# arneschneuing/DiffSBDD

Hardware: AMD Instinct MI355X
Metric: sampled ligands/sec (500-step DDPM, fullatom_cond) at 1/2/4/8 MI355X (higher is better)
Workload: dtype f32

## Files before the change

### diffsbdd_amd/_lib.py

```python
from __future__ import annotations

import ctypes as C
import os

_HERE = os.path.dirname(os.path.abspath(__file__))
LIB_PATH = os.environ.get("DSBDD_LIB") or os.path.join(_HERE, "libdiffsbdd_hip.so")
ABI_VERSION = 6

OK, ERR_ARG, ERR_STATE, ERR_CAPACITY, ERR_LAUNCH = 0, -1, -2, -3, -4
STATUS_NAN, STATUS_EDGE_OVERFLOW = 1, 2

G_NAMES = ["ATOM_ENC_W0T", "ATOM_ENC_B0", "ATOM_ENC_W1T", "ATOM_ENC_B1",
           "RES_ENC_W0T", "RES_ENC_B0", "RES_ENC_W1T", "RES_ENC_B1",
           "ATOM_DEC_W0T", "ATOM_DEC_B0", "ATOM_DEC_W1T", "ATOM_DEC_B1",
           "RES_DEC_W0T", "RES_DEC_B0", "RES_DEC_W1T", "RES_DEC_B1",
           "EMB_WT", "EMB_B", "EMBOUT_WT", "EMBOUT_B"]
GCL_NAMES = ["E1_WT", "E1_WD", "E1_WD0", "E1_TAB", "E2_WT", "E2_B", "ATT_W", "ATT_B",
             "N1_WT", "N1_B", "N2_WT", "N2_B"]
EQ_NAMES = ["C1_WT", "C_WD", "C_WD0", "C_TAB", "C_W2T", "C_B2",
            "X_WD", "X_WD0", "X_TAB", "X_W2T", "X_B2", "W3"]
OPT_PRUNE, OPT_CONE, OPT_GRANULE16, OPT_EMU, OPT_SPLITK, OPT_SHELL, OPT_TAIL = 0, 1, 2, 3, 4, 5, 6
(BUF_EDGE_ROW, BUF_EDGE_COL, BUF_EDGE_D0, BUF_ROW_PTR, BUF_H, BUF_X, BUF_NODE_BATCH, BUF_DEG,
 BUF_LEVEL, BUF_LEVEL_LIST, BUF_LEVEL_COUNT, BUF_LEVEL_END, BUF_LROW_PTR, BUF_LEDGE_ROW, BUF_LEDGE_COL,
 BUF_LEDGE_D0, BUF_LEVEL_STATS) = range(17)


class Config(C.Structure):
    _fields_ = [(n, C.c_int32) for n in (
        "atom_nf", "residue_nf", "joint_nf", "hidden_nf", "n_layers", "inv_sublayers",
        "attention", "use_tanh", "update_pocket_coords", "reflection_equivariant",
        "edge_embedding_dim", "has_cutoff_ligand", "has_cutoff_pocket",
        "has_cutoff_interaction")] + [(n, C.c_float) for n in (
            "cutoff_ligand", "cutoff_pocket", "cutoff_interaction",
            "norm_constant", "normalization_factor", "coords_range")]


# ... 33 lines not shown
    "dsbdd_last_error": (C.c_char_p, []),
    "dsbdd_engine_create": (C.c_int, [C.POINTER(Config), C.POINTER(_P)]),
    "dsbdd_engine_destroy": (None, [_P]),
    "dsbdd_engine_weight_slots": (C.c_int, [_P]),
    "dsbdd_engine_set_weights": (C.c_int, [_P, C.POINTER(_P), C.c_int]),
    "dsbdd_engine_workspace_bytes": (C.c_size_t, [_P, _I64, _I64, _I64, _I64]),
    "dsbdd_engine_bind_workspace": (C.c_int, [_P, _P, C.c_size_t, _I64, _I64, _I64, _I64]),
    "dsbdd_engine_set_trace": (C.c_int, [_P, _P, _P]),
    "dsbdd_engine_set_pocket_frame": (C.c_int, [_P, _P, _P, _P, _P, _P, _I64, _I64, _I64, _I64, _I64, _I64]),
    "dsbdd_engine_clear_pocket_frame": (C.c_int, [_P]),
    "dsbdd_dynamics_forward": (C.c_int, [_P, _P, _P, _P, _P, _I64, _P, _P, _I64, _I64, _I64,
                                         _P, _P, _I64, _P, _P, _P]),
    "dsbdd_engine_buffer": (C.c_int, [_P, C.c_int, C.POINTER(_P)]),
    "dsbdd_engine_shell_read": (C.c_int, [_P, C.c_int, C.c_int, _P, C.c_int64]),
    "dsbdd_engine_graph_stats": (C.c_int, [_P, C.POINTER(_I64), C.POINTER(_I64), C.POINTER(_I64)]),
    "dsbdd_engine_last_plan": (C.c_int, [_P, C.POINTER(C.c_int32), C.POINTER(C.c_int32), C.c_int32,
                                         C.POINTER(C.c_int32), C.POINTER(C.c_int32)]),
    "dsbdd_engine_set_option": (C.c_int, [_P, C.c_int, C.c_int]),
    "dsbdd_engine_get_option": (C.c_int, [_P, C.c_int]),
    "dsbdd_engine_profile": (C.c_int, [_P, C.c_int, C.c_int]),
    "dsbdd_engine_profile_read": (C.c_int, [_P, C.POINTER(C.c_double), C.POINTER(_I64)]),
    "dsbdd_cond_reverse_update": (C.c_int, [_P, _P, _P, _P, _P, _P, _P, _I64, _I64, _I64,
                                            _I32, _I32, _F, _F, _F, _I32]),
    "dsbdd_joint_reverse_update": (C.c_int, [_P, _P, _P, _P, _P, _P, _P, _P, _P, _I64, _I64, _I64,
                                             _I32, _I32, _F, _F, _F, _I32]),
    "dsbdd_segment_mean3": (C.c_int, [_P, _P, _I32, _P, _I64, _I64, _P]),
    "dsbdd_cond_affine_noise": (C.c_int, [_P, _P, _P, _P, _P, _P, _I64, _I64, _I64, _I32, _I32, _F, _F, _I32]),
    "dsbdd_joint_affine_noise": (C.c_int, [_P, _P, _P, _P, _P, _P, _P, _I64, _I64, _I64, _I32, _I32, _F, _F,
                                           _I32, _I32]),
    "dsbdd_cond_repaint_update": (C.c_int, [_P, _P, _P, _P, _P, _P, _P, _P, _P, _P, _P, _I64, _I64, _I64,
# ... 109 lines not shown
```

### diffsbdd_amd/csrc/engine.hip

```cpp
#include "../../include/diffsbdd_hip.h"

#include <algorithm>
#include <climits>
#include <cmath>
#include <cstdio>
#include <cstdlib>
#include <cstring>
#include <string>
#include <type_traits>
#include <utility>
#include <vector>

#include "common.h"
#include "ddpm.h"
#include "edge_mlp.h"
#include "edge_wave.h"
#include "edge_wave16.h"
#include "edge_splitk.h"
#include "graph.h"
#include "lig_head.h"
#include "ligand_pack.h"
#include "molecule.h"
#include "node_chain.h"
#include "node_linear.h"
// ... 79 lines not shown
int dsbdd_engine_bind_workspace(dsbdd_engine* e, void* ws, size_t bytes, int64_t nl, int64_t np,
                                int64_t B, int64_t E) {
  if (!e || !ws) return fail(DSBDD_ERR_ARG, "null argument");
  if (reinterpret_cast<uintptr_t>(ws) & 255) return fail(DSBDD_ERR_ARG, "workspace must be 256-byte aligned");
  if ((nl + np) >= (1ll << 30) || E >= (1ll << 31) - 256) return fail(DSBDD_ERR_ARG, "problem too large for int32 indices");
  if (bytes < ws_carve(e->cfg, nl, np, B, E, nullptr).total) return fail(DSBDD_ERR_CAPACITY, "workspace too small");
  e->drop_graphs();
  static_cast<Workspace&>(*e) = ws_carve(e->cfg, nl, np, B, E, static_cast<char*>(ws));
  e->ws = static_cast<char*>(ws); e->ws_bytes = bytes;
  e->cap_lig = nl; e->cap_poc = np; e->cap_batch = B; e->cap_edges = E;
  e->cap_edgesL = 2 * E + 32 * kLevels * B;
  e->cap_tiles = e->cap_edgesL / 32 + 2;
  e->cap_shell = E + 32 * B;
  e->cap_tiles16 = e->cap_edgesL / 16 + 2;
  e->lvl_stats_zeroed = false;
  e->frame = false;
  e->ghost_dirty = true;
  e->h0_pocket_valid = false;
  e->invalidate_derived();
  return DSBDD_OK;
}

#ifdef DSBDD_TIMESTAMPS
int dsbdd_debug_set_timestamps(dsbdd_engine* e, unsigned long long* buf, int capacity) {
  if (!e) return DSBDD_ERR_ARG;
  e->ts_buf = buf; e->ts_cap = capacity; e->ts_next = 0;
  return DSBDD_OK;
}
#endif

// ... 59 lines not shown

int dsbdd_engine_set_option(dsbdd_engine* e, int which, int value) {
  if (!e) return fail(DSBDD_ERR_ARG, "null argument");
  switch (which) {
    case DSBDD_OPT_PRUNE: e->prune = value ? 1 : 0; break;
    case DSBDD_OPT_CONE: e->cone = value <= 0 ? 0 : (value >= 2 ? 2 : 1); break;
    case DSBDD_OPT_GRANULE16: e->granule16 = (unsigned)value; break;
    case DSBDD_OPT_SPLITK: e->splitk = (unsigned)value; break;
    case DSBDD_OPT_EMU:
      if (value != 0 && value != 6 && value != 9) return fail(DSBDD_ERR_ARG, "DSBDD_OPT_EMU takes 0, 6 or 9");
      e->emu = value; break;
    case DSBDD_OPT_SHELL: e->shell = value ? 1 : 0; break;
    case DSBDD_OPT_TAIL:
      if (value < 0) return fail(DSBDD_ERR_ARG, "DSBDD_OPT_TAIL takes a value >= 0");
      e->tail = value; break;
    default: return fail(DSBDD_ERR_ARG, "unknown option");
  }
  e->drop_graphs();
  return DSBDD_OK;
}

int dsbdd_engine_get_option(const dsbdd_engine* e, int which) {
  if (!e) return fail(DSBDD_ERR_ARG, "null argument");
  switch (which) {
    case DSBDD_OPT_PRUNE: return e->prune;
    case DSBDD_OPT_CONE: return e->cone;
    case DSBDD_OPT_GRANULE16: return (int)e->granule16;
    case DSBDD_OPT_SPLITK: return (int)e->splitk;
    case DSBDD_OPT_EMU: return e->emu;
    case DSBDD_OPT_SHELL: return e->shell;
    case DSBDD_OPT_TAIL: return e->tail;
  }
  return fail(DSBDD_ERR_ARG, "unknown option");
}

int dsbdd_engine_set_trace(dsbdd_engine* e, float* th, float* tx) {
  if (!e) return DSBDD_ERR_ARG;
  e->trace_h = th; e->trace_x = tx;
  return DSBDD_OK;
}

int dsbdd_engine_profile(dsbdd_engine* e, int enable, int max_launches) {
  if (!e || max_launches < 0) return fail(DSBDD_ERR_ARG, "bad argument");
  e->profile = enable < 0 ? 0 : enable;
  e->prof_call = 0;
  e->ev_used = 0;
// ... 21 lines not shown
}

int dsbdd_engine_graph_stats(const dsbdd_engine* e, int64_t* replays, int64_t* captures, int64_t* eager) {
  if (!e || !replays || !captures || !eager) return fail(DSBDD_ERR_ARG, "null argument");
  *replays = e->n_replay; *captures = e->n_capture; *eager = e->n_eager;
  return DSBDD_OK;
}

int dsbdd_engine_buffer(const dsbdd_engine* e, int which, void** out) {
  if (!e || !out || !e->ws) return fail(DSBDD_ERR_STATE, "no workspace bound");
  void* const buf[] = {e->erow, e->ecol, e->ed0, e->row_ptr, e->h, e->x, e->node_batch, e->deg, e->lvl, e->lvl_list, e->lvl_cnt,
                       e->lvl_end, e->row_ptrL, e->erowL, e->ecolL, e->ed0L, e->lvl_stats};
  static_assert(DSBDD_BUF_LEVEL_STATS + 1 == sizeof(buf) / sizeof(buf[0]), "one pointer per DSBDD_BUF_* id");
  if (which < 0 || which > DSBDD_BUF_LEVEL_STATS) return fail(DSBDD_ERR_ARG, "unknown buffer id");
  *out = buf[which];
  return DSBDD_OK;
}

int dsbdd_engine_shell_read(const dsbdd_engine* e, int which, int list, void* dst, int64_t count) {
  if (!e || !dst || count < 0) return fail(DSBDD_ERR_ARG, "bad argument");
  if (!e->shell_mem) return fail(DSBDD_ERR_STATE, "no shell stage has run on this engine");
  const int64_t N = e->shell_key[0], SL = e->shell_key[2];
  const void* src = nullptr;
  int64_t have = 0, size = 4;
  const bool lst = list >= 0 && list < kShellLists;
  switch (which) {
    case DSBDD_SHELL_STATS: src = e->sh_stats; have = 8; size = 8; break;
    case DSBDD_SHELL_COUNT: src = e->sh_cnt; have = kShellLists; break;
    case DSBDD_SHELL_ROW: if (lst) { src = e->sh_row + (size_t)list * SL; have = SL; } break;
    case DSBDD_SHELL_COL: if (lst) { src = e->sh_col + (size_t)list * SL; have = SL; } break;
// ... 41 lines not shown
```

### diffsbdd_amd/csrc/engine_state.h

```cpp
#pragma once

static thread_local std::string g_err;
static int fail(int code, const std::string& msg) { g_err = msg; return code; }

#define HIP_TRY(expr)                                                              \
  do {                                                                             \
    hipError_t _e = (expr);                                                        \
    if (_e != hipSuccess)                                                          \
      return fail(DSBDD_ERR_LAUNCH, std::string(#expr) + ": " + hipGetErrorString(_e)); \
  } while (0)
#define RC_TRY(expr)                       \
  do {                                     \
    const int _rc = (expr);                \
    if (_rc != DSBDD_OK) return _rc;       \
  } while (0)

struct StreamDevice {
  int prev = -1;
  bool switched = false;
  explicit StreamDevice(void* stream) {
    hipStream_t s = static_cast<hipStream_t>(stream);
    if (!s) return;
    hipDevice_t d = 0;
    int cur = 0;
// ... 111 lines not shown

struct dsbdd_engine : Workspace {
  dsbdd_config cfg;
  std::vector<const float*> slots;
  bool has_weights = false;
  char* ws = nullptr;
  size_t ws_bytes = 0;
  int64_t cap_lig = 0, cap_poc = 0, cap_batch = 0, cap_edges = 0;
  bool lvl_stats_zeroed = false;
  int64_t cap_edgesL = 0;
  int prune = 1;
  int cone = 1;
  int64_t ghost_slots = 0;
  int shell = 1;
  int tail = 1;
  int64_t cap_shell = 0;
  char* shell_mem = nullptr;
  int64_t shell_key[3] = {0, 0, 0};
  int *sh_seg = nullptr, *sh_deg = nullptr, *sh_ptr = nullptr, *sh_row = nullptr, *sh_col = nullptr, *sh_cnt = nullptr;
  float* sh_d0 = nullptr;
  unsigned long long* sh_stats = nullptr;
  float* msg_buf = nullptr;
  int64_t msg_cap = 0;
  std::vector<int> plan_radius, plan_ghost;
  int plan_timed_level = kLevels - 1;
  bool frame = false;
  int64_t frame_nlig = 0, frame_npoc = 0, frame_batch = 0, frame_n3 = 0, frame_cap3 = 0;
  bool ghost_dirty = true;
  bool h0_pocket_valid = false;
  int64_t cap_tiles = 0;
// ... 21 lines not shown
  struct GraphEntry {
    std::vector<uint64_t> key;
    int seen = 0;
    hipGraph_t graph = nullptr;
    hipGraphExec_t exec = nullptr;
    std::vector<int> plan_radius, plan_ghost;
    int plan_timed_level = 0;
    void destroy() { if (exec) (void)hipGraphExecDestroy(exec); if (graph) (void)hipGraphDestroy(graph); }
  };
  std::vector<GraphEntry> graphs;
  int use_graph = 1;
  int coord_split = 1;
  int node_group = 1;
  int edge_max_wg = 0;
  int64_t n_replay = 0, n_capture = 0, n_eager = 0;
  unsigned long long* ts_buf = nullptr;
  int ts_cap = 0, ts_next = 0;
  hipStream_t cap_stream = nullptr;
  dsbdd_engine() : Workspace{} {}
  void drop_graphs() {
    for (GraphEntry& g : graphs) g.destroy();
    graphs.clear();
  }
  void invalidate_derived() { derived = DerivedReady{}; }
  ~dsbdd_engine() {
    for (hipEvent_t e : ev) (void)hipEventDestroy(e);
    drop_graphs();
    if (cap_stream) (void)hipStreamDestroy(cap_stream);
    if (side_stream) (void)hipStreamDestroy(side_stream);
    if (ev_fork) (void)hipEventDestroy(ev_fork);
// ... 62 lines not shown
  const std::pair<const char*, int*> off_on_zero[] = {
      {"DSBDD_GRAPH", &e->use_graph}, {"DSBDD_EDGE_BPERM", &e->edge_bperm}, {"DSBDD_COORD_SPLIT", &e->coord_split},
      {"DSBDD_NODE_GROUP", &e->node_group}, {"DSBDD_PRUNE", &e->prune}, {"DSBDD_LIG_HEAD", &e->lig_head},
      {"DSBDD_NODE_CHAIN", &e->chain}};
  for (const auto& sw : off_on_zero) if (env_int(sw.first, &v) && v == 0) *sw.second = 0;
  const std::pair<const char*, int*> on_nonzero[] = {{"DSBDD_LEVEL_ROWS", &e->level_rows}, {"DSBDD_FORK", &e->fork_front}};
  for (const auto& sw : on_nonzero) if (env_int(sw.first, &v)) *sw.second = v != 0;
  if (env_int("DSBDD_FOLD_SCAN", &v)) e->fold_scan = v > 0 ? 1 : 0;
  if (env_int("DSBDD_GRANULE16", &v, true)) e->granule16 = (unsigned)v;
  if (env_int("DSBDD_SPLITK", &v, true)) e->splitk = (unsigned)v;
  if (env_int("DSBDD_EMU", &v)) e->emu = (v == 6 || v == 9) ? (int)v : 0;
  if (env_int("DSBDD_CONE", &v)) e->cone = v <= 0 ? 0 : (v >= 2 ? 2 : 1);
  if (env_int("DSBDD_NODE_CHAIN_MIN_ROWS", &v) && v >= 0) e->chain_min_rows = v;
  if (env_int("DSBDD_EDGE_MAX_WG", &v) && v > 0) e->edge_max_wg = (int)v;
  if (env_int("DSBDD_TAIL", &v) && v >= 0) e->tail = (int)v;
}
```

### diffsbdd_amd/csrc/forward.h

```cpp
#pragma once

struct ForwardArgs {
  const float *xh_lig, *xh_pocket, *t;
  int64_t t_count;
  const int64_t *mask_lig, *mask_pocket;
  int64_t n_lig, n_pocket, batch;
  const int32_t *ext_row, *ext_col;
  int64_t ext_n_edges;
  float *eps_lig, *eps_pocket;
  int32_t* status;
};

static bool frame_applies(const dsbdd_engine* e, const ForwardArgs& a) {
  return e->frame && !e->cfg.update_pocket_coords && !a.ext_row && a.n_lig == e->frame_nlig &&
         a.n_pocket == e->frame_npoc && a.batch == e->frame_batch;
}

static Mlp2Problem residue_encoder(const dsbdd_engine* e, const ForwardArgs& a) {
  const dsbdd_config& c = e->cfg;
  const int r = c.residue_nf, J = c.joint_nf, JP = pad4(J + 1);
  const float* const* W = e->slots.data();
  return Mlp2Problem{a.xh_pocket + 3, 3 + r, r, W[DSBDD_G_RES_ENC_W0T], pad4(2 * r), W[DSBDD_G_RES_ENC_B0], 2 * r,
                     W[DSBDD_G_RES_ENC_W1T], pad4(J), W[DSBDD_G_RES_ENC_B1], J, e->h0 + (size_t)a.n_lig * JP, JP,
                     (int)a.n_pocket};
// ... 18 lines not shown
  const int PQ = (c.reflection_equivariant ? 2 : 4) * H;
  const float* const* W = e->slots.data();
  const bool subset = !c.update_pocket_coords;

  const bool split0 = frame_applies(e, *this);
  const bool prune = e->prune && subset && !ext && !eps_pocket && !e->trace_h && !e->trace_x && nlig > 0;
  const int G_stages = c.n_layers * c.inv_sublayers;
  const bool cone_pays = e->cone >= 2 || 5 * e->frame_n3 <= 2 * (int64_t)n_pocket;
  const bool cone = prune && split0 && e->cone && cone_pays && t_count == 1 && G_stages >= 2;
  const int n_frame_rows = split0 ? (int)e->frame_n3 : 0;
  const int n_ghost = (split0 && prune) ? n_frame_rows : 0;
  const int64_t ghost_slots = (split0 && prune) ? e->ghost_slots : 0;
  static constexpr int LV = kLevels - 1;
  const int g_ghost_last = ghost_last();
  const bool fork = e->fork_front && !ext;
  hipStream_t sa = s;
  int64_t edge_bound = e->cap_edges;
  bool mean_in_levels = false;
  const int* L_row = prune ? e->erowL : e->erow;
  const int* L_col = prune ? e->ecolL : e->ecol;
  const float* L_d0 = prune ? e->ed0L : e->ed0;
  const int* L_ptr = prune ? e->row_ptrL : e->row_ptr;
  const int L_cap = prune ? (int)e->cap_edgesL : (int)e->cap_edges;
  int64_t L_bound() const { return prune ? e->cap_edgesL : edge_bound; }
  const int* act_rows = prune ? e->lvl_list + n_ghost : e->act_list;
  const int* act_count = prune ? e->lvl_cnt + kLevels + 1 : e->act_ptr + N;
  const int n_upd = c.update_pocket_coords ? N : nlig;
  const int* e_all = prune ? e->lvl_end + kLevels + LV : e->row_ptr + N;
  const int* e_upd = prune ? e->lvl_end + kLevels : e->row_ptr + n_upd;
  const bool can_sk = w2_enabled(e, W2_SPLITK);
// ... 89 lines not shown
          residue_encoder(e, *this)};
      if (mlp2_fits(enc[0]) && mlp2_fits(enc[1])) {
        HIP_TRY(launch_mlp2(sa, enc, (split0 && e->h0_pocket_valid) ? 1 : 2));
      } else {
        HIP_TRY(nl(sa, xh_lig + 3, dl, a, nullptr, 0, 0, W[DSBDD_G_ATOM_ENC_W0T], pad4(2 * a), W[DSBDD_G_ATOM_ENC_B0],
                   nullptr, 0, e->enc_tmp, LE, n_lig, 2 * a, 1));
        HIP_TRY(nl(sa, e->enc_tmp, LE, 2 * a, nullptr, 0, 0, W[DSBDD_G_ATOM_ENC_W1T], pad4(J),
                   W[DSBDD_G_ATOM_ENC_B1], nullptr, 0, e->h0, JP, n_lig, J, 0));
        float* tmp_p = e->enc_tmp + (size_t)n_lig * LE;
        HIP_TRY(nl(sa, xh_pocket + 3, dp, r, nullptr, 0, 0, W[DSBDD_G_RES_ENC_W0T], pad4(2 * r), W[DSBDD_G_RES_ENC_B0],
                   nullptr, 0, tmp_p, LE, n_pocket, 2 * r, 1));
        HIP_TRY(nl(sa, tmp_p, LE, 2 * r, nullptr, 0, 0, W[DSBDD_G_RES_ENC_W1T], pad4(J), W[DSBDD_G_RES_ENC_B1],
                   nullptr, 0, e->h0 + (size_t)n_lig * JP, JP, n_pocket, J, 0));
      }
    }
    HIP_TRY(nl(sa, e->h0, JP, JP, nullptr, 0, 0, W[DSBDD_G_EMB_WT], H, W[DSBDD_G_EMB_B], nullptr, 0, e->h, H, N, H, 0));
    if (split0) {
      hipLaunchKernelGGL(gather_rows_kernel, dim3((e->frame_n3 + 3) / 4), dim3(kThreads), 0, sa, e->h + (size_t)N * H,
                         (const float*)(e->h + (size_t)nlig * H), (const int*)e->frame_rows, (int)e->frame_n3, H);
      HIP_TRY(hipGetLastError());
    }
    if (fork) HIP_TRY(hipEventRecord(e->ev_join, sa));
    return DSBDD_OK;
  }

  int edge_list() {
    if (ext) {
      HIP_TRY(zero_async(e->deg, (size_t)N * 4, s));
      if (ext_n_edges > 0) {
        hipLaunchKernelGGL(ext_edges_kernel, dim3((int)((ext_n_edges + 255) / 256)), dim3(256), 0, s, ext_row,
                           ext_col, (int)ext_n_edges, (const float*)e->x, e->erow, e->ecol, e->ed0, e->deg);
        HIP_TRY(hipGetLastError());
      }
      hipLaunchKernelGGL(scan_kernel, dim3(1), dim3(1024), 0, s, (const int*)e->deg, e->row_ptr, N, SegAlign{},
                         (const int*)nullptr, (int*)nullptr, SegAlign{});
      HIP_TRY(hipGetLastError());
      edge_bound = ext_n_edges > 0 ? ext_n_edges : 1;
      if (subset) {
// ... 39 lines not shown
        if (cb > 2048) cb = 2048;
        if (cb < 1) cb = 1;
        hipLaunchKernelGGL(level_copy_kernel, dim3((int)cb), dim3(256), 0, s, la, N);
        HIP_TRY(hipGetLastError());
      }
    }
    if (subset && !prune) {
      hipLaunchKernelGGL(scan_kernel, dim3(1), dim3(1024), 0, s, (const int*)e->act_flag, e->act_ptr, N, SegAlign{},
                         (const int*)nullptr, (int*)nullptr, SegAlign{});
      HIP_TRY(hipGetLastError());
      hipLaunchKernelGGL(compact_kernel, dim3((N + 255) / 256), dim3(256), 0, s, (const int*)e->act_flag,
                         (const int*)e->act_ptr, e->act_list, N);
      HIP_TRY(hipGetLastError());
    }
    if (fork) HIP_TRY(hipStreamWaitEvent(s, e->ev_join, 0));
    return DSBDD_OK;
  }

  int derived_weights() {
    const int rc = w2_pack_missing(e, s);
    if (rc) return rc;
    if (use_chain && !e->derived.chain) {
      auto pack = [&](const float* WT, int ldw, int K, int Ncols, const float* dst) {
        hipLaunchKernelGGL(pack_b16_kernel, dim3((K * Ncols + 255) / 256), dim3(256), 0, s, WT, ldw, K, Ncols,
                           const_cast<float*>(dst));
      };
      for (int blk = 0; blk < c.n_layers; ++blk) {
        for (int sub = 0; sub < c.inv_sublayers; ++sub) {
          pack(W[gcl_slot(c, blk, sub, DSBDD_GCL_N1_WT)], H, 2 * H, H, chain_w(blk, sub, 0));
          pack(W[gcl_slot(c, blk, sub, DSBDD_GCL_N2_WT)], H, H, H, chain_w(blk, sub, 1));
// ... 133 lines not shown
        const bool same_rows = nx.row_idx == n1.row_idx && nx.m_count == n1.m_count && nx.M == n1.M;
        if (same_rows || ghost) {
          ca.proj[ca.n_proj++] = ChainProj{chain_w(nb, ns, 2), e->pqg, 2 * H, 2 * H, nullptr, 0};
          st.chained_pq = true;
          fill_pq = ghost && !same_rows;
        }
      }
      HIP_TRY(launch_node_chain(s, ca, H, e->n_cu));
    } else {
      HIP_TRY(launch_node_linear(s, n1));
      HIP_TRY(launch_node_linear(s, n2));
    }
    if (ghost) {
      const int hi = radius_of(g + 1) + 1 < LV ? radius_of(g + 1) + 1 : LV;
      if (hi > radius) {
        hipLaunchKernelGGL(canon_fill_kernel, dim3((N - nlig + 3) / 4), dim3(kThreads), 0, s, e->h,
                           (const int*)e->lvl, (const int*)e->twin, nlig, N, N, radius, hi, H,
                           fill_pq ? e->pqg : (float*)nullptr, 2 * H);
        HIP_TRY(hipGetLastError());
      }
    }
    return DSBDD_OK;
  }

  int coord_stage(int blk, StageState& st) {
    auto Q = [&](int which) { return W[eq_slot(c, blk, which)]; };
    const int QW = n_mlp * H;
    NodeLinearArgs grp[kMaxGroup];
    int ng = 0;
    if (!st.chained_coord) {
      if (subset) {
        grp[ng++] = NodeLinearArgs{e->h, H, H, nullptr, 0, 0, Q(DSBDD_EQ_C1_WT), PQ, nullptr, nullptr, 0, e->pq, PQ,
// ... 141 lines not shown
```

### diffsbdd_amd/csrc/graph.h

```cpp
#pragma once
#include "common.h"

namespace dsbdd {

constexpr int kTileCtrInts = 32;
constexpr int kEdgeAlign = 32;
constexpr int kLevels = 5;
constexpr int kShellLists = 2;

struct Cutoffs {
  int has_l, has_p, has_i;
  float cl, cp, ci;
};

__device__ __forceinline__ int lower_bound_i64(const int64_t* a, int n, int64_t v) {
  int lo = 0, hi = n;
  while (lo < hi) {
    const int mid = (lo + hi) >> 1;
    if (a[mid] < v) lo = mid + 1; else hi = mid;
  }
  return lo;
}

__global__ void prep_kernel(const int64_t* mask_lig, int n_lig, const int64_t* mask_poc, int n_poc,
// ... 475 lines not shown
    x[3 * (id_dst + i)] = xframe[3 * i]; x[3 * (id_dst + i) + 1] = xframe[3 * i + 1];
    x[3 * (id_dst + i) + 2] = xframe[3 * i + 2];
  }
}

__global__ __launch_bounds__(kThreads) void gather_rows_kernel(float* dst, const float* src, const int* rows, int n,
                                                               int H) {
  const int i = (blockIdx.x * kThreads + threadIdx.x) >> 6, lane = threadIdx.x & 63;
  if (i >= n) return;
  const float* a = src + (size_t)rows[i] * H;
  float* b = dst + (size_t)i * H;
  for (int k = 4 * lane; k < H; k += 256) *reinterpret_cast<float4*>(b + k) = ld4(a + k);
}

__global__ __launch_bounds__(kThreads) void canon_fill_kernel(float* h, const int* lvl, const int* twin_local,
                                                              int n_lig, int n_nodes, int ghost_base, int lo,
                                                              int hi, int H, float* pq = nullptr, int ldpq = 0) {
  const int i = n_lig + ((blockIdx.x * kThreads + threadIdx.x) >> 6), lane = threadIdx.x & 63;
  if (i >= n_nodes) return;
  const int L = lvl[i];
  if (L <= lo || L > hi) return;
  const int g = ghost_base + twin_local[i - n_lig];
  const float* src = h + (size_t)g * H;
  float* dst = h + (size_t)i * H;
  for (int k = 4 * lane; k < H; k += 256) *reinterpret_cast<float4*>(dst + k) = ld4(src + k);
  if (pq)
    for (int k = 4 * lane; k < ldpq; k += 256)
      *reinterpret_cast<float4*>(pq + (size_t)i * ldpq + k) = ld4(pq + (size_t)g * ldpq + k);
}

__global__ void level_copy_kernel(LevelArgs a, int n_nodes) {
  const int total = min(a.row_ptr_nat[n_nodes], a.e_cap_nat);
  for (int e = blockIdx.x * blockDim.x + threadIdx.x; e < total; e += gridDim.x * blockDim.x) {
    const int i = a.erow_nat[e];
    if (i < 0 || i >= n_nodes) continue;
    const int pos = a.row_ptr[i] + (e - a.row_ptr_nat[i]);
    if (pos >= 0 && pos < a.e_cap) { a.erow[pos] = i; a.ecol[pos] = a.ecol_nat[e]; a.ed0[pos] = a.ed0_nat[e]; }
    const int L = i >= a.n_lig ? a.lvl[i] : 0;
    if (L >= 2 && L - 2 < a.n_shell) {
      const int j = a.ecol_nat[e];
      if (j < a.n_lig || a.lvl[j] < L) {
        int rank = 0;
        for (int q = max(a.row_ptr_nat[i], 0); q < e; ++q) {
// ... 210 lines not shown
```

### diffsbdd_amd/csrc/graph_cache.h

```cpp
#pragma once

static int ghost_setup(dsbdd_engine* e, hipStream_t s) {
  const int n3 = (int)e->frame_n3, N = (int)(e->frame_nlig + e->frame_npoc);
  int64_t gb = (e->frame_cap3 + 255) / 256;
  if (gb > 1024) gb = 1024;
  hipLaunchKernelGGL(ghost_setup_kernel, dim3((int)gb), dim3(256), 0, s, (const int*)e->erow3, (const int*)e->ecol3,
                     (const float*)e->ed03, (const int*)e->row_ptr3, (const int*)e->deg3, n3, N, N, e->erowL,
                     e->ecolL, e->ed0L, (int)e->cap_edgesL, e->deg, e->row_ptrL, e->lvl_list,
                     (const float*)e->xframe, e->x);
  HIP_TRY(hipGetLastError());
  e->ghost_dirty = false;
  return DSBDD_OK;
}

static int shell_memory(dsbdd_engine* e, hipStream_t s) {
  const int64_t N = e->cap_lig + e->cap_poc, B = e->cap_batch, SL = e->cap_shell;
  if (e->shell_mem && e->shell_key[0] == N && e->shell_key[1] == B && e->shell_key[2] == SL && e->msg_cap >= e->ghost_slots)
    return DSBDD_OK;
  HIP_TRY(hipStreamSynchronize(s));
  e->drop_graphs();
  if (e->shell_mem) (void)hipFree(e->shell_mem);
  e->shell_mem = nullptr; e->msg_cap = 0;
  auto lay = [&](Carver c) {
    auto ints = [&](size_t n) { return reinterpret_cast<int*>(c.bytes(n * 4)); };
// ... 10 lines not shown
  e->shell_key[0] = N; e->shell_key[1] = B; e->shell_key[2] = SL; e->msg_cap = e->ghost_slots;
  return DSBDD_OK;
}

static int frame_upkeep(dsbdd_engine* e, hipStream_t s, const ForwardArgs& a) {
  if (!frame_applies(e, a)) {
    e->ghost_dirty = true;
    e->h0_pocket_valid = false;
    return DSBDD_OK;
  }
  if (e->ghost_dirty) {
    int rc = ghost_setup(e, s);
    if (rc) return rc;
  }
  if (Forward(e, s, a).n_shell() > 0) RC_TRY(shell_memory(e, s));
  if (!e->h0_pocket_valid) {
    Mlp2Problem enc = residue_encoder(e, a);
    if (mlp2_fits(enc)) {
      HIP_TRY(launch_mlp2(s, &enc, 1));
      e->h0_pocket_valid = true;
    }
  }
  return DSBDD_OK;
}

static dsbdd_engine::GraphEntry* graph_entry(dsbdd_engine* e, hipStream_t s, const ForwardArgs& a) {
  std::vector<uint64_t> key = {(uint64_t)(uintptr_t)a.xh_lig, (uint64_t)(uintptr_t)a.xh_pocket, (uint64_t)(uintptr_t)a.t,
                               (uint64_t)a.t_count, (uint64_t)(uintptr_t)a.mask_lig, (uint64_t)(uintptr_t)a.mask_pocket,
                               (uint64_t)a.n_lig, (uint64_t)a.n_pocket, (uint64_t)a.batch, (uint64_t)(uintptr_t)a.eps_lig,
                               (uint64_t)(uintptr_t)a.eps_pocket, (uint64_t)(uintptr_t)a.status,
// ... 15 lines not shown
  HIP_TRY(hipStreamBeginCapture(e->cap_stream, hipStreamCaptureModeThreadLocal));
  const int rc = forward_impl(e, e->cap_stream, a);
  hipGraph_t graph = nullptr;
  hipGraphExec_t exec = nullptr;
  const hipError_t ec = hipStreamEndCapture(e->cap_stream, &graph);
  const bool ok = rc == DSBDD_OK && ec == hipSuccess && graph &&
                  hipGraphInstantiate(&exec, graph, nullptr, nullptr, 0) == hipSuccess && exec;
  if (!ok) {
    if (graph) (void)hipGraphDestroy(graph);
    e->use_graph = 0;
    e->derived = before;
    return rc;
  }
  g->graph = graph;
  g->exec = exec;
  g->plan_radius = e->plan_radius; g->plan_ghost = e->plan_ghost; g->plan_timed_level = e->plan_timed_level;
  return DSBDD_OK;
}

static int forward_cached(dsbdd_engine* e, hipStream_t s, const ForwardArgs& a) {
  dsbdd_engine::GraphEntry* g = graph_entry(e, s, a);
  if (g->exec) {
    ++e->n_replay;
    HIP_TRY(hipGraphLaunch(g->exec, s));
    e->plan_radius = g->plan_radius; e->plan_ghost = g->plan_ghost; e->plan_timed_level = g->plan_timed_level;
    return DSBDD_OK;
  }
  ++e->n_eager;
  if (g->seen++ == 0) return forward_impl(e, s, a);
  if (!e->cap_stream) HIP_TRY(hipStreamCreateWithFlags(&e->cap_stream, hipStreamNonBlocking));
// ... 8 lines not shown
```

### diffsbdd_amd/csrc/node_linear.h

```cpp
#pragma once
#include "common.h"

namespace dsbdd {

struct NodeLinearArgs {
  const float* A1; int lda1; int K1;
  const float* A2; int lda2; int K2;
  const float* WT; int ldw;
  const float* bias;
  const float* R; int ldr;
  float* C; int ldc;
  int M; int N; int act;
  const int* row_idx; const int* m_count;
};

template <int BM, bool VEC_A>
__global__ __launch_bounds__(kThreads) void node_linear_kernel(NodeLinearArgs p) {
  constexpr int BN = 128, BK = 32, LDA = BM + 1;
  constexpr int RT = BM / 64;
  constexpr int AI = BM / 32;
  __shared__ float sA[BK * LDA];
  __shared__ float sB[BK * BN];

  const int t = threadIdx.x, lane = t & 63, w = t >> 6;
  const int wm = w >> 1, wn = w & 1;
  const int m0 = blockIdx.x * BM, n0 = blockIdx.y * BN;
  const int K = p.K1 + p.K2;
  const int M = p.m_count ? min(p.M, *p.m_count) : p.M;
  if (m0 >= M) return;

  f32x16 acc[RT][2];
#pragma unroll
  for (int i = 0; i < RT; ++i)
#pragma unroll
    for (int j = 0; j < 2; ++j)
#pragma unroll
      for (int r = 0; r < 16; ++r) acc[i][j][r] = 0.f;

  float4 ra[AI], rb[4];
  const int a_kq = (t & 7) * 4, a_m = t >> 3;
  const int b_n = (t & 31) * 4, b_k = t >> 5;

  auto gload = [&](int k0) {
#pragma unroll
    for (int i = 0; i < AI; ++i) {
      const int ml = m0 + a_m + 32 * i, k = k0 + a_kq;
      float4 v = make_float4(0.f, 0.f, 0.f, 0.f);
      if (ml < M) {
        const int m = p.row_idx ? p.row_idx[ml] : ml;
        if (VEC_A) {
          if (k < K) {
            const float* src = (k < p.K1) ? p.A1 + (size_t)m * p.lda1 + k
                                          : p.A2 + (size_t)m * p.lda2 + (k - p.K1);
            v = ld4(src);
          }
        } else {
          float e[4];
#pragma unroll
          for (int c = 0; c < 4; ++c) {
            const int kk = k + c;
            e[c] = 0.f;
            if (kk < K)
              e[c] = (kk < p.K1) ? p.A1[(size_t)m * p.lda1 + kk]
                                 : p.A2[(size_t)m * p.lda2 + (kk - p.K1)];
// ... 51 lines not shown
    }
    __syncthreads();
  }

#pragma unroll
  for (int i = 0; i < RT; ++i) {
#pragma unroll
    for (int j = 0; j < 2; ++j) {
      const int col = n0 + wn * 64 + j * 32 + (lane & 31);
      if (col >= p.N) continue;
      const float bv = p.bias ? p.bias[col] : 0.f;
#pragma unroll
      for (int r = 0; r < 16; ++r) {
        const int rowl = m0 + wm * (BM / 2) + i * 32 + mfma_row(r, lane);
        if (rowl >= M) continue;
        const int row = p.row_idx ? p.row_idx[rowl] : rowl;
        float v = acc[i][j][r] + bv;
        if (p.act == 1) v = silu(v);
        if (p.R) v += p.R[(size_t)row * p.ldr + col];
        p.C[(size_t)row * p.ldc + col] = v;
      }
    }
  }
}


constexpr int kMaxGroup = 3;
struct NodeGroupArgs { NodeLinearArgs p[kMaxGroup]; };

#ifndef DSBDD_NODE_BK2
#define DSBDD_NODE_BK2 16
// ... 218 lines not shown
        hipDeviceGetAttribute(&cu, hipDeviceAttributeMultiprocessorCount, dev) != hipSuccess || cu <= 0)
      return 0;
    int p = 1;
    while (2 * p <= cu) p *= 2;
    return 2 * p;
  }();
  return v;
}

inline hipError_t launch_node_group(hipStream_t s, const NodeLinearArgs* a, int n) {
  if (n <= 0 || n > kMaxGroup) return hipErrorInvalidValue;
  bool all_small = true;
  for (int i = 0; i < n; ++i) all_small = all_small && gemm_ct(a[i], node_ct_override()) == 1;
  int ct = 4;
  for (int i = 0; i < n; ++i) {
    const int c = gemm_ct(a[i], node_ct_override(), all_small);
    if (c == 0) return hipErrorInvalidValue;
    if (c < ct) ct = c;
  }
  for (int i = 0; i < n; ++i)
    if (gemm_ct(a[i], ct) != ct) return hipErrorInvalidValue;
  NodeGroupArgs ga{};
  int balance = ct > 1 ? node_balance() : 0;
  for (int i = 0; i < n && balance > 0; ++i)
    if (gemm_ct(a[i], ct / 2) != ct / 2 || balance % (a[i].N / (32 * ct)) != 0) balance = 0;
  int gx = 0;
  for (int i = 0; i < n; ++i) {
    ga.p[i] = a[i];
    gx = max(gx, ((a[i].M + 127) / 128) * (a[i].N / (32 * ct)) * (balance > 0 ? 2 : 1));
  }
  dim3 grid(gx, 1, n), block(kThreads);
  if (ct == 4)      hipLaunchKernelGGL((node_gemm_kernel<4>), grid, block, 0, s, ga, balance);
  else if (ct == 2) hipLaunchKernelGGL((node_gemm_kernel<2>), grid, block, 0, s, ga, balance);
  else              hipLaunchKernelGGL((node_gemm_kernel<1>), grid, block, 0, s, ga, balance);
  return hipGetLastError();
}

inline hipError_t launch_node_linear(hipStream_t s, const NodeLinearArgs& a) {
  if (a.M <= 0 || a.N <= 0) return hipSuccess;
  const bool vec = vec_ok(a);
  if ((long)a.M * a.N >= 64 * 1024 && gemm_ct(a, node_ct_override()) != 0) return launch_node_group(s, &a, 1);
  const int ny = (a.N + 127) / 128;
  const long tiles128 = (long)((a.M + 127) / 128) * ny;
  const bool big = tiles128 >= 512 && !a.row_idx;
  const int bm = big ? 128 : 64;
  dim3 grid((a.M + bm - 1) / bm, ny), block(kThreads);
  if (big) {
    if (vec) hipLaunchKernelGGL((node_linear_kernel<128, true>), grid, block, 0, s, a);
    else     hipLaunchKernelGGL((node_linear_kernel<128, false>), grid, block, 0, s, a);
  } else {
    if (vec) hipLaunchKernelGGL((node_linear_kernel<64, true>), grid, block, 0, s, a);
    else     hipLaunchKernelGGL((node_linear_kernel<64, false>), grid, block, 0, s, a);
  }
  return hipGetLastError();
}

}
```

### diffsbdd_amd/engine.py

```python
from __future__ import annotations

import ctypes as C

import torch

from . import _lib


def _pad4(v):
    return (v + 3) & ~3


def make_config(atom_nf, residue_nf, joint_nf, hidden_nf, n_layers, inv_sublayers, attention,
                tanh, update_pocket_coords, reflection_equivariant, edge_embedding_dim,
                edge_cutoff_ligand, edge_cutoff_pocket, edge_cutoff_interaction, norm_constant,
                normalization_factor, coords_range=15.0):
    cfg = _lib.Config()
    cfg.atom_nf, cfg.residue_nf, cfg.joint_nf, cfg.hidden_nf = atom_nf, residue_nf, joint_nf, hidden_nf
    cfg.n_layers, cfg.inv_sublayers = n_layers, inv_sublayers
    cfg.attention, cfg.use_tanh = int(bool(attention)), int(bool(tanh))
    cfg.update_pocket_coords = int(bool(update_pocket_coords))
    cfg.reflection_equivariant = int(bool(reflection_equivariant))
    cfg.edge_embedding_dim = int(edge_embedding_dim or 0)
    for name, v in (("ligand", edge_cutoff_ligand), ("pocket", edge_cutoff_pocket),
# ... 256 lines not shown
        return eps_lig, eps_pocket, status

    def profile(self, enable, max_launches=16384):
        _lib.check(self.lib.dsbdd_engine_profile(self.handle, int(enable), int(max_launches)))

    def profile_read(self):
        ms, n = C.c_double(0), C.c_int64(0)
        _lib.check(self.lib.dsbdd_engine_profile_read(self.handle, C.byref(ms), C.byref(n)))
        return ms.value, n.value

    def graph_stats(self):
        r, c, g = C.c_int64(0), C.c_int64(0), C.c_int64(0)
        _lib.check(self.lib.dsbdd_engine_graph_stats(self.handle, C.byref(r), C.byref(c), C.byref(g)))
        return r.value, c.value, g.value

    def edge_count(self, n_nodes):
        import numpy as np
        torch.cuda.synchronize(self.device)
        return int(self._read(self.buffer_ptr(_lib.BUF_DEG), n_nodes, np.int32).astype(np.int64).sum())

    def edge_slots(self, n_nodes):
        import numpy as np
        torch.cuda.synchronize(self.device)
        return int(self._read(self.buffer_ptr(_lib.BUF_ROW_PTR) + 4 * n_nodes, 1, np.int32)[0])

    def buffer_ptr(self, which):
        p = C.c_void_p()
        _lib.check(self.lib.dsbdd_engine_buffer(self.handle, which, C.byref(p)))
        return p.value

# ... 66 lines not shown
```

### include/diffsbdd_hip.h

```cpp
#ifndef DIFFSBDD_HIP_H
#define DIFFSBDD_HIP_H

#include <stddef.h>
#include <stdint.h>

#ifdef __cplusplus
extern "C" {
#endif

#define DSBDD_ABI_VERSION 6

enum {
  DSBDD_OK = 0,
  DSBDD_ERR_ARG = -1,
  DSBDD_ERR_STATE = -2,
  DSBDD_ERR_CAPACITY = -3,
  DSBDD_ERR_LAUNCH = -4
};

enum {
  DSBDD_STATUS_NAN = 1,
  DSBDD_STATUS_EDGE_OVERFLOW = 2
};

// ... 65 lines not shown
int dsbdd_engine_clear_pocket_frame(dsbdd_engine* e);

int dsbdd_engine_set_trace(dsbdd_engine* e, float* trace_h, float* trace_x);

int dsbdd_dynamics_forward(dsbdd_engine* e, void* stream, const float* xh_lig,
                           const float* xh_pocket, const float* t, int64_t t_count,
                           const int64_t* mask_lig, const int64_t* mask_pocket, int64_t n_lig,
                           int64_t n_pocket, int64_t batch, const int32_t* ext_row,
                           const int32_t* ext_col, int64_t ext_n_edges, float* eps_lig,
                           float* eps_pocket, int32_t* status);

int dsbdd_engine_profile(dsbdd_engine* e, int enable, int max_launches);
int dsbdd_engine_profile_read(dsbdd_engine* e, double* total_ms, int64_t* launches);

int dsbdd_engine_graph_stats(const dsbdd_engine* e, int64_t* replays, int64_t* captures, int64_t* eager);

int dsbdd_engine_last_plan(const dsbdd_engine* e, int32_t* radius, int32_t* ghost, int32_t capacity,
                           int32_t* n_stages, int32_t* timed_level);

enum { DSBDD_OPT_PRUNE = 0, DSBDD_OPT_CONE = 1, DSBDD_OPT_GRANULE16 = 2, DSBDD_OPT_EMU = 3, DSBDD_OPT_SPLITK = 4,
       DSBDD_OPT_SHELL = 5, DSBDD_OPT_TAIL = 6 };
int dsbdd_engine_set_option(dsbdd_engine* e, int which, int value);
int dsbdd_engine_get_option(const dsbdd_engine* e, int which);

enum {
  DSBDD_BUF_EDGE_ROW = 0, DSBDD_BUF_EDGE_COL, DSBDD_BUF_EDGE_D0, DSBDD_BUF_ROW_PTR,
  DSBDD_BUF_H, DSBDD_BUF_X, DSBDD_BUF_NODE_BATCH, DSBDD_BUF_DEG,
  DSBDD_BUF_LEVEL, DSBDD_BUF_LEVEL_LIST, DSBDD_BUF_LEVEL_COUNT, DSBDD_BUF_LEVEL_END,
  DSBDD_BUF_LROW_PTR, DSBDD_BUF_LEDGE_ROW, DSBDD_BUF_LEDGE_COL, DSBDD_BUF_LEDGE_D0,
  DSBDD_BUF_LEVEL_STATS
};
int dsbdd_engine_buffer(const dsbdd_engine* e, int which, void** ptr_out);

enum { DSBDD_SHELL_STATS = 0, DSBDD_SHELL_COUNT, DSBDD_SHELL_ROW, DSBDD_SHELL_COL, DSBDD_SHELL_PTR, DSBDD_SHELL_DEG };
int dsbdd_engine_shell_read(const dsbdd_engine* e, int which, int list, void* dst, int64_t count);

int dsbdd_cond_reverse_update(void* stream, float* z_lig, float* xh_pocket, const float* eps_lig,
                              const float* noise, const int64_t* mask_lig,
                              const int64_t* mask_pocket, int64_t n_lig, int64_t n_pocket,
                              int64_t batch, int32_t atom_nf, int32_t residue_nf, float alpha_ts,
                              float c_eps, float sigma, int32_t remove_com);

int dsbdd_joint_reverse_update(void* stream, float* z_lig, float* z_pocket, const float* eps_lig,
                               const float* eps_pocket, const float* noise_lig,
                               const float* noise_pocket, const int64_t* mask_lig,
                               const int64_t* mask_pocket, int64_t n_lig, int64_t n_pocket,
                               int64_t batch, int32_t atom_nf, int32_t residue_nf, float alpha_ts,
// ... 214 lines not shown
```

Before: 41.53.

## Restrict embedding and ghost fills to rows actually read by later stages

Adds a READ_ROWS option mask (default 5) that, under cone pruning, makes the embedding linear run only over rows in the first stage's radius plus the frame rows. The embedding launch moves after edge-list construction so those rows are known. Ghost-level canon fills now take per-level masks for h, p and q, so copies that no later stage reads are skipped. To keep rows that are never written well defined, h and pq are zeroed once per workspace, and a debug query for graph node count is added. The row-selection logic is intricate and could leave stale data in rows if the reach analysis is wrong.

```diff
diff --git a/diffsbdd_amd/_lib.py b/diffsbdd_amd/_lib.py
--- a/diffsbdd_amd/_lib.py
+++ b/diffsbdd_amd/_lib.py
@@ -19,7 +19,7 @@
              "N1_WT", "N1_B", "N2_WT", "N2_B"]
 EQ_NAMES = ["C1_WT", "C_WD", "C_WD0", "C_TAB", "C_W2T", "C_B2",
             "X_WD", "X_WD0", "X_TAB", "X_W2T", "X_B2", "W3"]
-OPT_PRUNE, OPT_CONE, OPT_GRANULE16, OPT_EMU, OPT_SPLITK, OPT_SHELL, OPT_TAIL = 0, 1, 2, 3, 4, 5, 6
+OPT_PRUNE, OPT_CONE, OPT_GRANULE16, OPT_EMU, OPT_SPLITK, OPT_SHELL, OPT_TAIL, OPT_READ_ROWS = 0, 1, 2, 3, 4, 5, 6, 7
 (BUF_EDGE_ROW, BUF_EDGE_COL, BUF_EDGE_D0, BUF_ROW_PTR, BUF_H, BUF_X, BUF_NODE_BATCH, BUF_DEG,
  BUF_LEVEL, BUF_LEVEL_LIST, BUF_LEVEL_COUNT, BUF_LEVEL_END, BUF_LROW_PTR, BUF_LEDGE_ROW, BUF_LEDGE_COL,
  BUF_LEDGE_D0, BUF_LEVEL_STATS) = range(17)
@@ -83,6 +83,8 @@
     "dsbdd_engine_buffer": (C.c_int, [_P, C.c_int, C.POINTER(_P)]),
     "dsbdd_engine_shell_read": (C.c_int, [_P, C.c_int, C.c_int, _P, C.c_int64]),
     "dsbdd_engine_graph_stats": (C.c_int, [_P, C.POINTER(_I64), C.POINTER(_I64), C.POINTER(_I64)]),
+    "dsbdd_engine_graph_nodes": (C.c_int, [_P, C.POINTER(_I64)]),
+    "dsbdd_engine_pq_buffer": (C.c_int, [_P, C.POINTER(_P)]),
     "dsbdd_engine_last_plan": (C.c_int, [_P, C.POINTER(C.c_int32), C.POINTER(C.c_int32), C.c_int32,
                                          C.POINTER(C.c_int32), C.POINTER(C.c_int32)]),
     "dsbdd_engine_set_option": (C.c_int, [_P, C.c_int, C.c_int]),
diff --git a/diffsbdd_amd/csrc/engine.hip b/diffsbdd_amd/csrc/engine.hip
--- a/diffsbdd_amd/csrc/engine.hip
+++ b/diffsbdd_amd/csrc/engine.hip
@@ -117,6 +117,7 @@
   e->cap_shell = E + 32 * B;
   e->cap_tiles16 = e->cap_edgesL / 16 + 2;
   e->lvl_stats_zeroed = false;
+  e->rows_zeroed = false;
   e->frame = false;
   e->ghost_dirty = true;
   e->h0_pocket_valid = false;
@@ -206,6 +207,9 @@
     case DSBDD_OPT_TAIL:
       if (value < 0) return fail(DSBDD_ERR_ARG, "DSBDD_OPT_TAIL takes a value >= 0");
       e->tail = value; break;
+    case DSBDD_OPT_READ_ROWS:
+      if (value < 0 || value > 7) return fail(DSBDD_ERR_ARG, "DSBDD_OPT_READ_ROWS takes a mask 0 .. 7");
+      e->read_rows = value; break;
     default: return fail(DSBDD_ERR_ARG, "unknown option");
   }
   e->drop_graphs();
@@ -222,6 +226,7 @@
     case DSBDD_OPT_EMU: return e->emu;
     case DSBDD_OPT_SHELL: return e->shell;
     case DSBDD_OPT_TAIL: return e->tail;
+    case DSBDD_OPT_READ_ROWS: return e->read_rows;
   }
   return fail(DSBDD_ERR_ARG, "unknown option");
 }
@@ -273,6 +278,18 @@
   static_assert(DSBDD_BUF_LEVEL_STATS + 1 == sizeof(buf) / sizeof(buf[0]), "one pointer per DSBDD_BUF_* id");
   if (which < 0 || which > DSBDD_BUF_LEVEL_STATS) return fail(DSBDD_ERR_ARG, "unknown buffer id");
   *out = buf[which];
+  return DSBDD_OK;
+}
+
+int dsbdd_engine_pq_buffer(const dsbdd_engine* e, void** out) {
+  if (!e || !out || !e->ws) return fail(DSBDD_ERR_STATE, "no workspace bound");
+  *out = e->pqg;
+  return DSBDD_OK;
+}
+
+int dsbdd_engine_graph_nodes(const dsbdd_engine* e, int64_t* nodes) {
+  if (!e || !nodes) return fail(DSBDD_ERR_ARG, "null argument");
+  *nodes = e->graph_nodes;
   return DSBDD_OK;
 }
 
diff --git a/diffsbdd_amd/csrc/engine_state.h b/diffsbdd_amd/csrc/engine_state.h
--- a/diffsbdd_amd/csrc/engine_state.h
+++ b/diffsbdd_amd/csrc/engine_state.h
@@ -149,6 +149,8 @@
   int64_t ghost_slots = 0;
   int shell = 1;
   int tail = 1;
+  int read_rows = 5;
+  bool rows_zeroed = false;
   int64_t cap_shell = 0;
   char* shell_mem = nullptr;
   int64_t shell_key[3] = {0, 0, 0};
@@ -200,6 +202,7 @@
   int node_group = 1;
   int edge_max_wg = 0;
   int64_t n_replay = 0, n_capture = 0, n_eager = 0;
+  int64_t graph_nodes = 0;
   unsigned long long* ts_buf = nullptr;
   int ts_cap = 0, ts_next = 0;
   hipStream_t cap_stream = nullptr;
@@ -292,4 +295,5 @@
   if (env_int("DSBDD_NODE_CHAIN_MIN_ROWS", &v) && v >= 0) e->chain_min_rows = v;
   if (env_int("DSBDD_EDGE_MAX_WG", &v) && v > 0) e->edge_max_wg = (int)v;
   if (env_int("DSBDD_TAIL", &v) && v >= 0) e->tail = (int)v;
-}
+  if (env_int("DSBDD_READ_ROWS", &v, true) && v >= 0 && v <= 7) e->read_rows = (int)v;
+}
diff --git a/diffsbdd_amd/csrc/forward.h b/diffsbdd_amd/csrc/forward.h
--- a/diffsbdd_amd/csrc/forward.h
+++ b/diffsbdd_amd/csrc/forward.h
@@ -56,6 +56,8 @@
   static constexpr int LV = kLevels - 1;
   const int g_ghost_last = ghost_last();
   const bool fork = e->fork_front && !ext;
+  const bool embed_rows = cone && (e->read_rows & 1) && !fork && radius_of(0) < LV;
+  const bool trim_fills = cone && (e->read_rows & 4);
   hipStream_t sa = s;
   int64_t edge_bound = e->cap_edges;
   bool mean_in_levels = false;
@@ -175,14 +177,49 @@
                    nullptr, 0, e->h0 + (size_t)n_lig * JP, JP, n_pocket, J, 0));
       }
     }
-    HIP_TRY(nl(sa, e->h0, JP, JP, nullptr, 0, 0, W[DSBDD_G_EMB_WT], H, W[DSBDD_G_EMB_B], nullptr, 0, e->h, H, N, H, 0));
-    if (split0) {
-      hipLaunchKernelGGL(gather_rows_kernel, dim3((e->frame_n3 + 3) / 4), dim3(kThreads), 0, sa, e->h + (size_t)N * H,
-                         (const float*)(e->h + (size_t)nlig * H), (const int*)e->frame_rows, (int)e->frame_n3, H);
-      HIP_TRY(hipGetLastError());
-    }
+    if (!embed_rows) RC_TRY(embedding(sa));
     if (fork) HIP_TRY(hipEventRecord(e->ev_join, sa));
     return DSBDD_OK;
+  }
+
+  int embedding(hipStream_t st) {
+    NodeLinearArgs all{e->h0, JP, JP, nullptr, 0, 0, W[DSBDD_G_EMB_WT], H, W[DSBDD_G_EMB_B], nullptr, 0, e->h, H,
+                       N, H, 0, nullptr, nullptr, nullptr, 0, 0};
+    if (!embed_rows) {
+      HIP_TRY(launch_node_linear(st, all));
+    } else {
+      NodeLinearArgs rd = all;
+      rows_of(radius_of(0), false, rd);
+      rd.M = N;
+      rd.row_idx2 = e->frame_rows; rd.M2 = (int)e->frame_n3; rd.row_off2 = nlig;
+      HIP_TRY(launch_node_linear(st, rd));
+    }
+    if (split0) {
+      hipLaunchKernelGGL(gather_rows_kernel, dim3((e->frame_n3 + 3) / 4), dim3(kThreads), 0, st, e->h + (size_t)N * H,
+                         (const float*)(e->h + (size_t)nlig * H), (const int*)e->frame_rows, (int)e->frame_n3, H);
+      HIP_TRY(hipGetLastError());
+    }
+    return DSBDD_OK;
+  }
+
+  struct FillMasks { int h, p, q; };
+  FillMasks fill_masks(int g, int lo, int hi, bool fill_pq) const {
+    FillMasks m{0, 0, 0};
+    for (int L = lo + 1; L <= hi; ++L) {
+      bool need_h = !(trim_fills && fill_pq), need_p = need_h;
+      if (!need_p) need_p = L <= radius_of(g + 1);
+      for (int k = g + 1; k < G_stages && !need_h; ++k) {
+        if (L <= radius_of(k)) { need_h = true; break; }
+        if (k <= g_ghost_last) {
+          const int hk = radius_of(k + 1) + 1 < LV ? radius_of(k + 1) + 1 : LV;
+          if (L <= hk) break;
+        } else if (k + 1 < G_stages && L <= radius_of(k + 1) + 1) {
+          need_h = true;
+        }
+      }
+      m.h |= (int)need_h << L; m.p |= (int)need_p << L; m.q |= 1 << L;
+    }
+    return m;
   }
 
   int edge_list() {
@@ -252,6 +289,7 @@
       HIP_TRY(hipGetLastError());
     }
     if (fork) HIP_TRY(hipStreamWaitEvent(s, e->ev_join, 0));
+    if (embed_rows) RC_TRY(embedding(s));
     return DSBDD_OK;
   }
 
@@ -415,8 +453,9 @@
     if (ghost) {
       const int hi = radius_of(g + 1) + 1 < LV ? radius_of(g + 1) + 1 : LV;
       if (hi > radius) {
+        const FillMasks fm = fill_masks(g, radius, hi, fill_pq);
         hipLaunchKernelGGL(canon_fill_kernel, dim3((N - nlig + 3) / 4), dim3(kThreads), 0, s, e->h,
-                           (const int*)e->lvl, (const int*)e->twin, nlig, N, N, radius, hi, H,
+                           (const int*)e->lvl, (const int*)e->twin, nlig, N, N, fm.h, fm.p, fm.q, H,
                            fill_pq ? e->pqg : (float*)nullptr, 2 * H);
         HIP_TRY(hipGetLastError());
       }
diff --git a/diffsbdd_amd/csrc/graph.h b/diffsbdd_amd/csrc/graph.h
--- a/diffsbdd_amd/csrc/graph.h
+++ b/diffsbdd_amd/csrc/graph.h
@@ -513,19 +513,28 @@
 }
 
 __global__ __launch_bounds__(kThreads) void canon_fill_kernel(float* h, const int* lvl, const int* twin_local,
-                                                              int n_lig, int n_nodes, int ghost_base, int lo,
-                                                              int hi, int H, float* pq = nullptr, int ldpq = 0) {
+                                                              int n_lig, int n_nodes, int ghost_base, int mask_h,
+                                                              int mask_p, int mask_q, int H, float* pq = nullptr,
+                                                              int ldpq = 0) {
   const int i = n_lig + ((blockIdx.x * kThreads + threadIdx.x) >> 6), lane = threadIdx.x & 63;
   if (i >= n_nodes) return;
   const int L = lvl[i];
-  if (L <= lo || L > hi) return;
+  if ((unsigned)L >= 31u || !(((mask_h | mask_p | mask_q) >> L) & 1)) return;
   const int g = ghost_base + twin_local[i - n_lig];
-  const float* src = h + (size_t)g * H;
-  float* dst = h + (size_t)i * H;
-  for (int k = 4 * lane; k < H; k += 256) *reinterpret_cast<float4*>(dst + k) = ld4(src + k);
-  if (pq)
-    for (int k = 4 * lane; k < ldpq; k += 256)
-      *reinterpret_cast<float4*>(pq + (size_t)i * ldpq + k) = ld4(pq + (size_t)g * ldpq + k);
+  if ((mask_h >> L) & 1) {
+    const float* src = h + (size_t)g * H;
+    float* dst = h + (size_t)i * H;
+    for (int k = 4 * lane; k < H; k += 256) *reinterpret_cast<float4*>(dst + k) = ld4(src + k);
+  }
+  if (pq) {
+    const int half = ldpq / 2;
+    const float* src = pq + (size_t)g * ldpq;
+    float* dst = pq + (size_t)i * ldpq;
+    if ((mask_p >> L) & 1)
+      for (int k = 4 * lane; k < half; k += 256) *reinterpret_cast<float4*>(dst + k) = ld4(src + k);
+    if ((mask_q >> L) & 1)
+      for (int k = half + 4 * lane; k < ldpq; k += 256) *reinterpret_cast<float4*>(dst + k) = ld4(src + k);
+  }
 }
 
 __global__ void level_copy_kernel(LevelArgs a, int n_nodes) {
diff --git a/diffsbdd_amd/csrc/graph_cache.h b/diffsbdd_amd/csrc/graph_cache.h
--- a/diffsbdd_amd/csrc/graph_cache.h
+++ b/diffsbdd_amd/csrc/graph_cache.h
@@ -48,6 +48,12 @@
     if (rc) return rc;
   }
   if (Forward(e, s, a).n_shell() > 0) RC_TRY(shell_memory(e, s));
+  if (e->read_rows && !e->rows_zeroed) {
+    const size_t rows = (size_t)(e->cap_lig + 2 * e->cap_poc), H = (size_t)e->cfg.hidden_nf;
+    HIP_TRY(hipMemsetAsync(e->h, 0, rows * H * 4, s));
+    HIP_TRY(hipMemsetAsync(e->pqg, 0, rows * 2 * H * 4, s));
+    e->rows_zeroed = true;
+  }
   if (!e->h0_pocket_valid) {
     Mlp2Problem enc = residue_encoder(e, a);
     if (mlp2_fits(enc)) {
@@ -93,6 +99,8 @@
   }
   g->graph = graph;
   g->exec = exec;
+  size_t n_nodes = 0;
+  e->graph_nodes = hipGraphGetNodes(graph, nullptr, &n_nodes) == hipSuccess ? (int64_t)n_nodes : 0;
   g->plan_radius = e->plan_radius; g->plan_ghost = e->plan_ghost; g->plan_timed_level = e->plan_timed_level;
   return DSBDD_OK;
 }
diff --git a/diffsbdd_amd/csrc/node_linear.h b/diffsbdd_amd/csrc/node_linear.h
--- a/diffsbdd_amd/csrc/node_linear.h
+++ b/diffsbdd_amd/csrc/node_linear.h
@@ -12,6 +12,7 @@
   float* C; int ldc;
   int M; int N; int act;
   const int* row_idx; const int* m_count;
+  const int* row_idx2; int M2; int row_off2;
 };
 
 template <int BM, bool VEC_A>
@@ -26,8 +27,13 @@
   const int wm = w >> 1, wn = w & 1;
   const int m0 = blockIdx.x * BM, n0 = blockIdx.y * BN;
   const int K = p.K1 + p.K2;
-  const int M = p.m_count ? min(p.M, *p.m_count) : p.M;
+  const int M1 = p.m_count ? min(p.M, *p.m_count) : p.M;
+  const int M = M1 + (p.row_idx2 ? p.M2 : 0);
   if (m0 >= M) return;
+  auto phys = [&](int ml) {
+    if (ml >= M1) return p.row_idx2[ml - M1] + p.row_off2;
+    return p.row_idx ? p.row_idx[ml] : ml;
+  };
 
   f32x16 acc[RT][2];
 #pragma unroll
@@ -47,7 +53,7 @@
       const int ml = m0 + a_m + 32 * i, k = k0 + a_kq;
       float4 v = make_float4(0.f, 0.f, 0.f, 0.f);
       if (ml < M) {
-        const int m = p.row_idx ? p.row_idx[ml] : ml;
+        const int m = phys(ml);
         if (VEC_A) {
           if (k < K) {
             const float* src = (k < p.K1) ? p.A1 + (size_t)m * p.lda1 + k
@@ -129,7 +135,7 @@
       for (int r = 0; r < 16; ++r) {
         const int rowl = m0 + wm * (BM / 2) + i * 32 + mfma_row(r, lane);
         if (rowl >= M) continue;
-        const int row = p.row_idx ? p.row_idx[rowl] : rowl;
+        const int row = phys(rowl);
         float v = acc[i][j][r] + bv;
         if (p.act == 1) v = silu(v);
         if (p.R) v += p.R[(size_t)row * p.ldr + col];
@@ -378,7 +384,7 @@
   for (int i = 0; i < n; ++i) all_small = all_small && gemm_ct(a[i], node_ct_override()) == 1;
   int ct = 4;
   for (int i = 0; i < n; ++i) {
-    const int c = gemm_ct(a[i], node_ct_override(), all_small);
+    const int c = a[i].row_idx2 ? 0 : gemm_ct(a[i], node_ct_override(), all_small);
     if (c == 0) return hipErrorInvalidValue;
     if (c < ct) ct = c;
   }
@@ -403,12 +409,13 @@
 inline hipError_t launch_node_linear(hipStream_t s, const NodeLinearArgs& a) {
   if (a.M <= 0 || a.N <= 0) return hipSuccess;
   const bool vec = vec_ok(a);
-  if ((long)a.M * a.N >= 64 * 1024 && gemm_ct(a, node_ct_override()) != 0) return launch_node_group(s, &a, 1);
+  const int rows = a.M + (a.row_idx2 ? a.M2 : 0);
+  if ((long)a.M * a.N >= 64 * 1024 && !a.row_idx2 && gemm_ct(a, node_ct_override()) != 0) return launch_node_group(s, &a, 1);
   const int ny = (a.N + 127) / 128;
   const long tiles128 = (long)((a.M + 127) / 128) * ny;
   const bool big = tiles128 >= 512 && !a.row_idx;
   const int bm = big ? 128 : 64;
-  dim3 grid((a.M + bm - 1) / bm, ny), block(kThreads);
+  dim3 grid((rows + bm - 1) / bm, ny), block(kThreads);
   if (big) {
     if (vec) hipLaunchKernelGGL((node_linear_kernel<128, true>), grid, block, 0, s, a);
     else     hipLaunchKernelGGL((node_linear_kernel<128, false>), grid, block, 0, s, a);
diff --git a/diffsbdd_amd/engine.py b/diffsbdd_amd/engine.py
--- a/diffsbdd_amd/engine.py
+++ b/diffsbdd_amd/engine.py
@@ -294,6 +294,16 @@
         _lib.check(self.lib.dsbdd_engine_graph_stats(self.handle, C.byref(r), C.byref(c), C.byref(g)))
         return r.value, c.value, g.value
 
+    def graph_nodes(self):
+        n = C.c_int64(0)
+        _lib.check(self.lib.dsbdd_engine_graph_nodes(self.handle, C.byref(n)))
+        return n.value
+
+    def pq_buffer_ptr(self):
+        p = C.c_void_p()
+        _lib.check(self.lib.dsbdd_engine_pq_buffer(self.handle, C.byref(p)))
+        return p.value
+
     def edge_count(self, n_nodes):
         import numpy as np
         torch.cuda.synchronize(self.device)
diff --git a/include/diffsbdd_hip.h b/include/diffsbdd_hip.h
--- a/include/diffsbdd_hip.h
+++ b/include/diffsbdd_hip.h
@@ -103,12 +103,13 @@
 int dsbdd_engine_profile_read(dsbdd_engine* e, double* total_ms, int64_t* launches);
 
 int dsbdd_engine_graph_stats(const dsbdd_engine* e, int64_t* replays, int64_t* captures, int64_t* eager);
+int dsbdd_engine_graph_nodes(const dsbdd_engine* e, int64_t* nodes);
 
 int dsbdd_engine_last_plan(const dsbdd_engine* e, int32_t* radius, int32_t* ghost, int32_t capacity,
                            int32_t* n_stages, int32_t* timed_level);
 
 enum { DSBDD_OPT_PRUNE = 0, DSBDD_OPT_CONE = 1, DSBDD_OPT_GRANULE16 = 2, DSBDD_OPT_EMU = 3, DSBDD_OPT_SPLITK = 4,
-       DSBDD_OPT_SHELL = 5, DSBDD_OPT_TAIL = 6 };
+       DSBDD_OPT_SHELL = 5, DSBDD_OPT_TAIL = 6, DSBDD_OPT_READ_ROWS = 7 };
 int dsbdd_engine_set_option(dsbdd_engine* e, int which, int value);
 int dsbdd_engine_get_option(const dsbdd_engine* e, int which);
 
@@ -120,6 +121,7 @@
   DSBDD_BUF_LEVEL_STATS
 };
 int dsbdd_engine_buffer(const dsbdd_engine* e, int which, void** ptr_out);
+int dsbdd_engine_pq_buffer(const dsbdd_engine* e, void** ptr_out);
 
 enum { DSBDD_SHELL_STATS = 0, DSBDD_SHELL_COUNT, DSBDD_SHELL_ROW, DSBDD_SHELL_COL, DSBDD_SHELL_PTR, DSBDD_SHELL_DEG };
 int dsbdd_engine_shell_read(const dsbdd_engine* e, int which, int list, void* dst, int64_t count);
```

New measurement: 41.64, median of 6. About the same (+0.3%).
